# GatorSense/HyperPRI

Hardware: AMD Instinct MI355X
Metric: HSI cubes/sec (608x968x238) fwd+bwd (higher is better)
Workload: dtype f32; 1 GPU; CubeNET-64 n_channels=238 HSI 608x968 fp32, per-GPU batch 2, train mode, BCEWithLogits, fwd+bwd; global_batch=2, parallelism=dp1

## Files before the change

### hyperpri_amd/csrc/conv_wino.hip

```cpp
#include "common.h"

extern "C" size_t hpri_wino_packed_floats(int K, int Ncols_pad) { return (size_t)hpri_cdiv(K, 8) * 16 * 8 * Ncols_pad; }

struct WinoWgradArgs {
  const float* x; int x_cs, x_coff, x_cvalid;
  const float* dy; int dy_cs, dy_coff, dy_cvalid;
  float* ws;
  int N, H, W, Cr, Nr, cblk;
  int strips_x, strips_y, total, per_split;
  int ntile, items, per_xcd;
  int kw;
};

#define WG_XROW 36
#define WG_X_BYTES (4 * WG_XROW * 256)
#define WG_Y_BYTES (2 * 32 * 256)
#define WG_STAGE_BYTES (WG_X_BYTES + WG_Y_BYTES)

__global__ __launch_bounds__(512, 2) void conv_wino_wgrad_kernel(WinoWgradArgs a) {
  __shared__ __attribute__((aligned(1024))) unsigned char smem[2 * WG_STAGE_BYTES];
  const int tid = threadIdx.x, lane = tid & 63, wave = __builtin_amdgcn_readfirstlane(tid >> 6);
  const int li = lane & 31, lh = lane >> 5;
  const int fa = wave >> 1, fb = wave & 1;
  const int item = (int)(blockIdx.x & 7) * a.per_xcd + (int)(blockIdx.x >> 3);
  if (item >= a.items) return;
  const int split = item / a.ntile, tile = item - split * a.ntile;
  const int cb = tile % a.cblk, nbk = tile / a.cblk;
  const int c_blk = cb * 64, n_blk = nbk * 64;
  const int u0 = split * a.per_split, u1 = min(a.total, u0 + a.per_split);

  const int r1 = (fa == 0) ? 0 : 1, r2 = (fa == 3) ? 3 : 2;
  const float s1 = (fa == 2) ? -1.f : 1.f, s2 = (fa == 1 || fa == 2) ? 1.f : -1.f;
  const int c0 = fb;
  const float sigma = s1 * s2;

  f32x16 acc[2][2][2];
#pragma unroll
  for (int e = 0; e < 2; ++e)
#pragma unroll
    for (int ct = 0; ct < 2; ++ct)
#pragma unroll
      for (int nt = 0; nt < 2; ++nt)
#pragma unroll
        for (int r = 0; r < 16; ++r) acc[e][ct][nt][r] = 0.f;

  constexpr int NPX = 4 * (WG_XROW / 4), NPY = 2 * 8, NPW = (NPX + NPY + 7) / 8;
  constexpr unsigned OOB = 0xFFFFFFF0u;
  const int l4 = lane >> 4;
  const unsigned xlane = (c_blk + (lane & 15) * 4 < a.x_cvalid) ? (unsigned)(l4 * a.x_cs * 4 + (lane & 15) * 16) : OOB;
  const unsigned ylane = (n_blk + (lane & 15) * 4 < a.dy_cvalid) ? (unsigned)(l4 * a.dy_cs * 4 + (lane & 15) * 16) : OOB;
#define LOAD_UNIT(u_, buf_)                                                                                            \
  {                                                                                                                    \
    int q_ = (u_);                                                                                                     \
    const int sx_ = q_ % a.strips_x; q_ /= a.strips_x;                                                                 \
    const int sy_ = q_ % a.strips_y; const int img_ = q_ / a.strips_y;                                                 \
    const int y0_ = sy_ * 2, x0_ = sx_ * 32;                                                                           \
    kend_next = min(8, (a.kw - x0_ + 3) >> 2);                                \
    unsigned char* lb_ = smem + (buf_) * WG_STAGE_BYTES;                                                               \
    const float* xu_ = a.x + ((long long)(img_ * a.H + y0_ - 1) * a.W + x0_ - 1) * a.x_cs + a.x_coff + c_blk;          \
    const float* yu_ = a.dy + ((long long)(img_ * a.H + y0_) * a.W + x0_) * a.dy_cs + a.dy_coff + n_blk;               \
    const hpri_rsrc_t rx_ = HPRI_MAKE_RSRC(xu_, 0x7FFFFF00);       \
    const hpri_rsrc_t ry_ = HPRI_MAKE_RSRC(yu_, 0x7FFFFF00);       \
    _Pragma("unroll") for (int p = 0; p < NPW; ++p) {                                                                  \
      const int piece_ = p * 8 + wave;                                                                                 \
      if (piece_ < NPX) {                                                                                              \
        const int row_ = piece_ / (WG_XROW / 4), pxb_ = (piece_ % (WG_XROW / 4)) * 4;                 \
        const bool rowok_ = (unsigned)(y0_ + row_ - 1) < (unsigned)a.H;                                                \
        const bool ok_ = rowok_ && (pxb_ + l4) < 34 && (unsigned)(x0_ + pxb_ + l4 - 1) < (unsigned)a.W;                \
        HPRI_LDS_DMA16(rx_, lb_ + piece_ * 1024, ok_ ? xlane : OOB, (row_ * a.W + pxb_) * a.x_cs * 4);           \
      } else if (piece_ < NPX + NPY) {                                                                                 \
        const int pp_ = piece_ - NPX;                                                                                  \
        const int row_ = pp_ >> 3, pxb_ = (pp_ & 7) * 4;                                                               \
        const bool ok_ = (y0_ + row_) < a.H && (x0_ + pxb_ + l4) < a.W;                                                \
        HPRI_LDS_DMA16(ry_, lb_ + piece_ * 1024, ok_ ? ylane : OOB, (row_ * a.W + pxb_) * a.dy_cs * 4);          \
      }                                                                                                                \
    }                                                                                                                  \
  }

#define K_STEP(FA_, FB_)                                               \
    {                                                                                                                  \
      const int tile = 2 * kk + lh;                                                                                    \
      float va[2][2], vb[2][2];                                               \
      _Pragma("unroll") for (int ct = 0; ct < 2; ++ct) {                                                               \
        float P[3];                                                                                                    \
        _Pragma("unroll") for (int c = 0; c < 3; ++c) {                                                                \
          const float d1 = xs[(r1 * WG_XROW + 2 * tile + c0 + c) * 64 + ct * 32 + li];                                 \
          const float d2 = xs[(r2 * WG_XROW + 2 * tile + c0 + c) * 64 + ct * 32 + li];                                 \
          P[c] = d1 + sigma * d2;                                                                                      \
        }                                                                                                              \
        va[0][ct] = FB_ ? (P[1] - P[0]) : (P[0] - P[2]);                                                               \
        va[1][ct] = FB_ ? (P[0] - P[2]) : (P[1] + P[2]);                                                               \
      }                                                                                                                \
      _Pragma("unroll") for (int nt = 0; nt < 2; ++nt) {                                                               \
        float t0, t1;                                                                                                  \
        if (FA_ == 0 || FA_ == 3) {                                                                                    \
          t0 = ys[(((FA_ == 3) ? 1 : 0) * 32 + 2 * tile + 0) * 64 + nt * 32 + li];                                     \
          t1 = ys[(((FA_ == 3) ? 1 : 0) * 32 + 2 * tile + 1) * 64 + nt * 32 + li];                                     \
        } else {                                                                                                       \
          const float y00 = ys[(0 * 32 + 2 * tile + 0) * 64 + nt * 32 + li], y01 = ys[(0 * 32 + 2 * tile + 1) * 64 + nt * 32 + li]; \
          const float y10 = ys[(1 * 32 + 2 * tile + 0) * 64 + nt * 32 + li], y11 = ys[(1 * 32 + 2 * tile + 1) * 64 + nt * 32 + li]; \
          t0 = (FA_ == 1) ? (y00 + y10) : (y00 - y10);                                                                 \
          t1 = (FA_ == 1) ? (y01 + y11) : (y01 - y11);                                                                 \
        }                                                                                                              \
        vb[0][nt] = FB_ ? (t0 - t1) : t0;                                                                              \
        vb[1][nt] = FB_ ? t1 : (t0 + t1);                                                                              \
      }                                                                                                                \
      _Pragma("unroll") for (int e = 0; e < 2; ++e)                                                                    \
          _Pragma("unroll") for (int ct = 0; ct < 2; ++ct)                                                             \
              _Pragma("unroll") for (int nt = 0; nt < 2; ++nt)                                                         \
                  acc[e][ct][nt] = __builtin_amdgcn_mfma_f32_32x32x2f32(va[e][ct], vb[e][nt], acc[e][ct][nt], 0, 0, 0); \
    }
#define UNIT_LOOP(FA_, FB_)                                                                                            \
  for (int u = u0; u < u1; ++u) {                                                                                      \
    asm volatile("s_waitcnt vmcnt(0)" ::: "memory");                                                                   \
    __builtin_amdgcn_s_barrier();                     \
    const int kend = kend_next;                                                                                        \
    if (u + 1 < u1) LOAD_UNIT(u + 1, (u + 1 - u0) & 1)                                                                 \
    const float* xs = reinterpret_cast<const float*>(smem + ((u - u0) & 1) * WG_STAGE_BYTES);                          \
    const float* ys = xs + WG_X_BYTES / 4;                                                                             \
    _Pragma("unroll 2") for (int kk = 0; kk < kend; ++kk) K_STEP(FA_, FB_)                                             \
  }
  int kend_next = 8;
  if (u0 < u1) LOAD_UNIT(u0, 0)
  switch (wave) {
    case 0: UNIT_LOOP(0, 0) break;
    case 1: UNIT_LOOP(0, 1) break;
    case 2: UNIT_LOOP(1, 0) break;
    case 3: UNIT_LOOP(1, 1) break;
    case 4: UNIT_LOOP(2, 0) break;
    case 5: UNIT_LOOP(2, 1) break;
    case 6: UNIT_LOOP(3, 0) break;
    default: UNIT_LOOP(3, 1) break;
  }
#undef UNIT_LOOP
#undef K_STEP
#undef LOAD_UNIT
  float* slab = a.ws + (size_t)split * 16 * a.Cr * a.Nr;
  const float sdy = (fa == 3) ? -s1 : s1;
  const float sgn[2] = {sdy, (fb == 1) ? -sdy : sdy};
#pragma unroll
  for (int e = 0; e < 2; ++e) {
    const int xi = fa * 4 + 2 * fb + e;
#pragma unroll
    for (int ct = 0; ct < 2; ++ct)
#pragma unroll
      for (int nt = 0; nt < 2; ++nt) {
        const int n = n_blk + nt * 32 + li;
#pragma unroll
        for (int r = 0; r < 16; ++r) {
          const int c = c_blk + ct * 32 + (r & 3) + 8 * (r >> 2) + 4 * lh;
          slab[((size_t)xi * a.Cr + c) * a.Nr + n] = sgn[e] * acc[e][ct][nt][r];
        }
      }
  }
}

__global__ void wino_wgrad_reduce_kernel(const float* __restrict__ ws, float* __restrict__ dw, int splits, int Cr, int Nr,
                                         int Cin, int Cout, int accumulate) {
  const int n = blockIdx.x * 64 + (threadIdx.x & 63), c = blockIdx.y * 4 + (threadIdx.x >> 6);
  if (n >= Cout || c >= Cin) return;
  float u[16];
#pragma unroll
  for (int xi = 0; xi < 16; ++xi) u[xi] = 0.f;
  const size_t slab = (size_t)16 * Cr * Nr;
  for (int k = 0; k < splits; ++k) {
    const float* p = ws + (size_t)k * slab + (size_t)c * Nr + n;
#pragma unroll
    for (int xi = 0; xi < 16; ++xi) u[xi] += p[(size_t)xi * Cr * Nr];
  }
  float t[3][4];
#pragma unroll
  for (int j = 0; j < 4; ++j) {
    t[0][j] = u[0 * 4 + j] + 0.5f * (u[1 * 4 + j] + u[2 * 4 + j]);
    t[1][j] = 0.5f * (u[1 * 4 + j] - u[2 * 4 + j]);
    t[2][j] = 0.5f * (u[1 * 4 + j] + u[2 * 4 + j]) + u[3 * 4 + j];
  }
  float* o = dw + ((size_t)n * Cin + c) * 9;
#pragma unroll
  for (int i = 0; i < 3; ++i) {
    const float g0 = t[i][0] + 0.5f * (t[i][1] + t[i][2]), g1 = 0.5f * (t[i][1] - t[i][2]), g2 = 0.5f * (t[i][1] + t[i][2]) + t[i][3];
    o[i * 3 + 0] = accumulate ? o[i * 3 + 0] + g0 : g0;
    o[i * 3 + 1] = accumulate ? o[i * 3 + 1] + g1 : g1;
    o[i * 3 + 2] = accumulate ? o[i * 3 + 2] + g2 : g2;
  }
}

constexpr int wino_wide_cols(int S) { return S >= 16 ? 32 : 64; }

template <int S>
__global__ __launch_bounds__(wino_wide_cols(S) * S) void wino_wgrad_reduce_wide_kernel(const float* __restrict__ ws,
                                                                                       float* __restrict__ dw, int splits, int Cr,
                                                                                       int Nr, int Cin, int Cout, int accumulate) {
  constexpr int NC = wino_wide_cols(S);
  __shared__ float red[S - 1][16][NC];
  const int ln = threadIdx.x % NC, sl = threadIdx.x / NC;
  const int n = blockIdx.x * NC + ln, c = blockIdx.y;
  float u[16];
#pragma unroll
  for (int xi = 0; xi < 16; ++xi) u[xi] = 0.f;
  const size_t slab = (size_t)16 * Cr * Nr;
#pragma unroll 1
  for (int k = sl; k < splits; k += S) {
    const float* p = ws + (size_t)k * slab + (size_t)c * Nr + n;
#pragma unroll
    for (int xi = 0; xi < 16; ++xi) u[xi] += p[(size_t)xi * Cr * Nr];
  }
  if (sl > 0) {
#pragma unroll
    for (int xi = 0; xi < 16; ++xi) red[sl - 1][xi][ln] = u[xi];
  }
  __syncthreads();
  if (sl > 0 || n >= Cout) return;
#pragma unroll 2
  for (int q = 0; q < S - 1; ++q)
#pragma unroll
    for (int xi = 0; xi < 16; ++xi) u[xi] += red[q][xi][ln];
  float t[3][4];
#pragma unroll
  for (int j = 0; j < 4; ++j) {
    t[0][j] = u[0 * 4 + j] + 0.5f * (u[1 * 4 + j] + u[2 * 4 + j]);
    t[1][j] = 0.5f * (u[1 * 4 + j] - u[2 * 4 + j]);
    t[2][j] = 0.5f * (u[1 * 4 + j] + u[2 * 4 + j]) + u[3 * 4 + j];
  }
  float* o = dw + ((size_t)n * Cin + c) * 9;
#pragma unroll
  for (int i = 0; i < 3; ++i) {
    const float g0 = t[i][0] + 0.5f * (t[i][1] + t[i][2]), g1 = 0.5f * (t[i][1] - t[i][2]), g2 = 0.5f * (t[i][1] + t[i][2]) + t[i][3];
    o[i * 3 + 0] = accumulate ? o[i * 3 + 0] + g0 : g0;
    o[i * 3 + 1] = accumulate ? o[i * 3 + 1] + g1 : g1;
    o[i * 3 + 2] = accumulate ? o[i * 3 + 2] + g2 : g2;
  }
}

extern "C" int hpri_wino_wgrad_plan(int N, int H, int W, int Cin_pad, int Cout_pad, int* splits, int* Cr, int* Nr) {
  const int cblk = hpri_cdiv(Cin_pad, 64), nblk = hpri_cdiv(Cout_pad, 64);
  const int total = N * hpri_cdiv(H, 2) * hpri_cdiv(W, 32);
  *Cr = cblk * 64; *Nr = nblk * 64;
  const int tiles = cblk * nblk;
  auto plan = [&](int cus, int kmax, double tol) {
    int best = 1; double best_eff = 0.0;
    for (int k = 1; k <= kmax; ++k) {
      if (k > 1 && total / k < 8) break;
      const double per_cu = (double)tiles * k / (double)cus;
      double eff = per_cu / (double)((long long)(per_cu + 0.999999));
      if (per_cu < 1.0) eff = per_cu;
      if (eff > best_eff + tol + 1e-9) { best_eff = eff; best = k; }
    }
    return best;
  };
  int best = plan(256, 512, 0.0);
  const int reserve = hpri_option(5);
  if (reserve > 0) best = plan(256 - (reserve < 192 ? reserve : 192), 2 * best, 0.05);
  *splits = best;
  return HPRI_OK;
}

extern "C" int hpri_conv_wino_wgrad(const float* x, int x_cs, int x_coff, int x_cvalid, const float* dy, int dy_cs, int dy_coff,
                                    int dy_cvalid, float* ws, size_t ws_floats, int N, int H, int W, int Cin_pad, int Cout_pad,
                                    hipStream_t stream) {
  HPRI_REQUIRE(x && dy && ws, "conv_wino_wgrad: null pointer");
  HPRI_REQUIRE(N > 0 && H > 0 && W > 0 && Cin_pad > 0 && Cout_pad > 0, "conv_wino_wgrad: bad sizes");
  HPRI_REQUIRE(x_cs % 4 == 0 && x_coff % 4 == 0 && dy_cs % 4 == 0 && dy_coff % 4 == 0 && x_cvalid % 4 == 0 && dy_cvalid % 4 == 0,
               "conv_wino_wgrad: channel strides / offsets / valid counts must be multiples of 4");
  HPRI_REQUIRE(((uintptr_t)x & 15) == 0 && ((uintptr_t)dy & 15) == 0, "conv_wino_wgrad: pointers must be 16-byte aligned");
  HPRI_REQUIRE((long long)5 * W * x_cs * 4 < (1ll << 31) && (long long)3 * W * dy_cs * 4 < (1ll << 31),
               "conv_wino_wgrad: image rows too long for 32-bit buffer offsets");
  WinoWgradArgs a;
  a.x = x; a.x_cs = x_cs; a.x_coff = x_coff; a.x_cvalid = x_cvalid; a.dy = dy; a.dy_cs = dy_cs; a.dy_coff = dy_coff; a.dy_cvalid = dy_cvalid;
  a.ws = ws; a.N = N; a.H = H; a.W = W;
  int splits;
  hpri_wino_wgrad_plan(N, H, W, Cin_pad, Cout_pad, &splits, &a.Cr, &a.Nr);
  if ((size_t)splits * 16 * a.Cr * a.Nr > ws_floats) return hpri_set_error(HPRI_ERR_WORKSPACE, "conv_wino_wgrad: workspace too small");
  a.cblk = a.Cr / 64;
  a.strips_x = hpri_cdiv(W, 32); a.strips_y = hpri_cdiv(H, 2); a.total = N * a.strips_x * a.strips_y;
  a.per_split = hpri_cdiv(a.total, splits);
  a.ntile = a.cblk * (a.Nr / 64);
  a.items = splits * a.ntile; a.per_xcd = hpri_cdiv(a.items, 8);
  a.kw = hpri_option(6) != 0 ? W : a.strips_x * 32;
  dim3 grid((unsigned)(a.per_xcd * 8), 1u, 1u);
  hipLaunchKernelGGL(conv_wino_wgrad_kernel, grid, dim3(512), 0, stream, a);
  HPRI_CHECK_LAUNCH();
  return HPRI_OK;
}

extern "C" int hpri_wino_wgrad_reduce(const float* ws, float* dw, int N, int H, int W, int Cin, int Cin_pad, int Cout, int Cout_pad,
                                      int accumulate, hipStream_t stream) {
  HPRI_REQUIRE(ws && dw && Cin > 0 && Cout > 0, "wino_wgrad_reduce: bad arguments");
  int splits, Cr, Nr;
  hpri_wino_wgrad_plan(N, H, W, Cin_pad, Cout_pad, &splits, &Cr, &Nr);
  if (splits >= 64) {
    dim3 grid((unsigned)hpri_cdiv(Cout, wino_wide_cols(16)), (unsigned)Cin);
    hipLaunchKernelGGL(wino_wgrad_reduce_wide_kernel<16>, grid, dim3(wino_wide_cols(16) * 16), 0, stream, ws, dw, splits, Cr, Nr, Cin, Cout, accumulate);
  } else if (splits >= 8) {
    dim3 grid((unsigned)hpri_cdiv(Cout, 64), (unsigned)Cin);
    hipLaunchKernelGGL(wino_wgrad_reduce_wide_kernel<8>, grid, dim3(512), 0, stream, ws, dw, splits, Cr, Nr, Cin, Cout, accumulate);
  } else {
    dim3 grid((unsigned)hpri_cdiv(Cout, 64), (unsigned)hpri_cdiv(Cin, 4));
    hipLaunchKernelGGL(wino_wgrad_reduce_kernel, grid, dim3(256), 0, stream, ws, dw, splits, Cr, Nr, Cin, Cout, accumulate);
  }
  HPRI_CHECK_LAUNCH();
  return HPRI_OK;
}
```

Baseline: 65.72 cubes/s.

## Vectorize Winograd wgrad LDS reads with interleaved channel pairs and pinned scheduling

Reworks the Winograd weight-gradient inner step so each lane reads adjacent channel pairs from LDS as 8-byte vectors through a running byte pointer. The transform signs and row choices become compile-time constants per wave. Channels are remapped to interleaved pairs so the output slab can be written with paired stores, and strip indices are advanced incrementally instead of recomputed with divisions. Inline-asm pins and a sched_barrier fix the placement of the transform arithmetic before the MFMAs. The aim is fewer LDS instructions and less address arithmetic, at the risk of worse compiler scheduling or register pressure.

```diff
diff --git a/hyperpri_amd/csrc/conv_wino.hip b/hyperpri_amd/csrc/conv_wino.hip
--- a/hyperpri_amd/csrc/conv_wino.hip
+++ b/hyperpri_amd/csrc/conv_wino.hip
@@ -1,4 +1,6 @@
 #include "common.h"
+
+typedef float f32x2 __attribute__((ext_vector_type(2)));
 
 extern "C" size_t hpri_wino_packed_floats(int K, int Ncols_pad) { return (size_t)hpri_cdiv(K, 8) * 16 * 8 * Ncols_pad; }
 
@@ -29,10 +31,7 @@
   const int c_blk = cb * 64, n_blk = nbk * 64;
   const int u0 = split * a.per_split, u1 = min(a.total, u0 + a.per_split);
 
-  const int r1 = (fa == 0) ? 0 : 1, r2 = (fa == 3) ? 3 : 2;
-  const float s1 = (fa == 2) ? -1.f : 1.f, s2 = (fa == 1 || fa == 2) ? 1.f : -1.f;
-  const int c0 = fb;
-  const float sigma = s1 * s2;
+  const float s1 = (fa == 2) ? -1.f : 1.f;
 
   f32x16 acc[2][2][2];
 #pragma unroll
@@ -49,11 +48,11 @@
   const int l4 = lane >> 4;
   const unsigned xlane = (c_blk + (lane & 15) * 4 < a.x_cvalid) ? (unsigned)(l4 * a.x_cs * 4 + (lane & 15) * 16) : OOB;
   const unsigned ylane = (n_blk + (lane & 15) * 4 < a.dy_cvalid) ? (unsigned)(l4 * a.dy_cs * 4 + (lane & 15) * 16) : OOB;
-#define LOAD_UNIT(u_, buf_)                                                                                            \
+  int ld_sx = u0 % a.strips_x, ld_sy = (u0 / a.strips_x) % a.strips_y, ld_img = u0 / (a.strips_x * a.strips_y);
+#define LOAD_UNIT(buf_)                                                                                                \
   {                                                                                                                    \
-    int q_ = (u_);                                                                                                     \
-    const int sx_ = q_ % a.strips_x; q_ /= a.strips_x;                                                                 \
-    const int sy_ = q_ % a.strips_y; const int img_ = q_ / a.strips_y;                                                 \
+    const int sx_ = ld_sx, sy_ = ld_sy, img_ = ld_img;                                                                 \
+    if (++ld_sx == a.strips_x) { ld_sx = 0; if (++ld_sy == a.strips_y) { ld_sy = 0; ++ld_img; } }                      \
     const int y0_ = sy_ * 2, x0_ = sx_ * 32;                                                                           \
     kend_next = min(8, (a.kw - x0_ + 3) >> 2);                                \
     unsigned char* lb_ = smem + (buf_) * WG_STAGE_BYTES;                                                               \
@@ -79,49 +78,72 @@
 
 #define K_STEP(FA_, FB_)                                               \
     {                                                                                                                  \
-      const int tile = 2 * kk + lh;                                                                                    \
+      constexpr int R1_ = (FA_ == 0) ? 0 : 1, R2_ = (FA_ == 3) ? 3 : 2;              \
+      constexpr int YR_ = (FA_ == 3) ? 1 : 0, YROWS_ = (FA_ == 1 || FA_ == 2) ? 2 : 1;                                 \
+      asm("" : "+v"(kp));                               \
+      f32x2 d[2][3], y[2][2];                                          \
+      _Pragma("unroll") for (int c = 0; c < 3; ++c) {                                                                  \
+        d[0][c] = WG_LDS2(kp + (R1_ * WG_XROW + FB_ + c) * 256);                                                       \
+        d[1][c] = WG_LDS2(kp + (R2_ * WG_XROW + FB_ + c) * 256);                                                       \
+      }                                                                                                                \
+      _Pragma("unroll") for (int r = 0; r < YROWS_; ++r)                                                               \
+        _Pragma("unroll") for (int px = 0; px < 2; ++px) y[r][px] = WG_LDS2(kp + WG_X_BYTES + ((YR_ + r) * 32 + px) * 256); \
       float va[2][2], vb[2][2];                                               \
+      float P[3][2];                                                                                                   \
+      _Pragma("unroll") for (int c = 0; c < 3; ++c)                                                                    \
+        _Pragma("unroll") for (int ct = 0; ct < 2; ++ct) {                                                             \
+          float d1_ = d[0][c][ct], d2_ = d[1][c][ct];                                                                  \
+          WG_PIN(d1_) WG_PIN(d2_)                                                                                      \
+          P[c][ct] = (FA_ == 1) ? (d1_ + d2_) : (d1_ - d2_);                                        \
+          WG_PIN(P[c][ct])                                                                                             \
+        }                                                                                                              \
       _Pragma("unroll") for (int ct = 0; ct < 2; ++ct) {                                                               \
-        float P[3];                                                                                                    \
-        _Pragma("unroll") for (int c = 0; c < 3; ++c) {                                                                \
-          const float d1 = xs[(r1 * WG_XROW + 2 * tile + c0 + c) * 64 + ct * 32 + li];                                 \
-          const float d2 = xs[(r2 * WG_XROW + 2 * tile + c0 + c) * 64 + ct * 32 + li];                                 \
-          P[c] = d1 + sigma * d2;                                                                                      \
+        va[0][ct] = FB_ ? (P[1][ct] - P[0][ct]) : (P[0][ct] - P[2][ct]);                                               \
+        va[1][ct] = FB_ ? (P[0][ct] - P[2][ct]) : (P[1][ct] + P[2][ct]);                                               \
+                                                                                                                       \
+      }                                                                                                                \
+      float t[2][2];                                                               \
+      _Pragma("unroll") for (int px = 0; px < 2; ++px)                                                                 \
+        _Pragma("unroll") for (int nt = 0; nt < 2; ++nt) {                                                             \
+          float y0_ = y[0][px][nt];                                                                                    \
+          WG_PIN(y0_)                                                                                                  \
+          if (YROWS_ == 2) {                                                                                           \
+            float y1_ = y[1][px][nt];                                                                                  \
+            WG_PIN(y1_)                                                                                                \
+            y0_ = (FA_ == 1) ? (y0_ + y1_) : (y0_ - y1_);                                                              \
+            WG_PIN(y0_)                                                                                                \
+          }                                                                                                            \
+          t[px][nt] = y0_;                                                                                             \
         }                                                                                                              \
-        va[0][ct] = FB_ ? (P[1] - P[0]) : (P[0] - P[2]);                                                               \
-        va[1][ct] = FB_ ? (P[0] - P[2]) : (P[1] + P[2]);                                                               \
+      _Pragma("unroll") for (int nt = 0; nt < 2; ++nt) {                                                               \
+        vb[0][nt] = FB_ ? (t[0][nt] - t[1][nt]) : t[0][nt];                                                            \
+        vb[1][nt] = FB_ ? t[1][nt] : (t[0][nt] + t[1][nt]);                                                            \
+                                                                                                                       \
       }                                                                                                                \
-      _Pragma("unroll") for (int nt = 0; nt < 2; ++nt) {                                                               \
-        float t0, t1;                                                                                                  \
-        if (FA_ == 0 || FA_ == 3) {                                                                                    \
-          t0 = ys[(((FA_ == 3) ? 1 : 0) * 32 + 2 * tile + 0) * 64 + nt * 32 + li];                                     \
-          t1 = ys[(((FA_ == 3) ? 1 : 0) * 32 + 2 * tile + 1) * 64 + nt * 32 + li];                                     \
-        } else {                                                                                                       \
-          const float y00 = ys[(0 * 32 + 2 * tile + 0) * 64 + nt * 32 + li], y01 = ys[(0 * 32 + 2 * tile + 1) * 64 + nt * 32 + li]; \
-          const float y10 = ys[(1 * 32 + 2 * tile + 0) * 64 + nt * 32 + li], y11 = ys[(1 * 32 + 2 * tile + 1) * 64 + nt * 32 + li]; \
-          t0 = (FA_ == 1) ? (y00 + y10) : (y00 - y10);                                                                 \
-          t1 = (FA_ == 1) ? (y01 + y11) : (y01 - y11);                                                                 \
-        }                                                                                                              \
-        vb[0][nt] = FB_ ? (t0 - t1) : t0;                                                                              \
-        vb[1][nt] = FB_ ? t1 : (t0 + t1);                                                                              \
-      }                                                                                                                \
+      __builtin_amdgcn_sched_barrier(0);                            \
       _Pragma("unroll") for (int e = 0; e < 2; ++e)                                                                    \
           _Pragma("unroll") for (int ct = 0; ct < 2; ++ct)                                                             \
               _Pragma("unroll") for (int nt = 0; nt < 2; ++nt)                                                         \
                   acc[e][ct][nt] = __builtin_amdgcn_mfma_f32_32x32x2f32(va[e][ct], vb[e][nt], acc[e][ct][nt], 0, 0, 0); \
+      kp += 1024;                                                                           \
     }
 #define UNIT_LOOP(FA_, FB_)                                                                                            \
   for (int u = u0; u < u1; ++u) {                                                                                      \
     asm volatile("s_waitcnt vmcnt(0)" ::: "memory");                                                                   \
     __builtin_amdgcn_s_barrier();                     \
     const int kend = kend_next;                                                                                        \
-    if (u + 1 < u1) LOAD_UNIT(u + 1, (u + 1 - u0) & 1)                                                                 \
-    const float* xs = reinterpret_cast<const float*>(smem + ((u - u0) & 1) * WG_STAGE_BYTES);                          \
-    const float* ys = xs + WG_X_BYTES / 4;                                                                             \
-    _Pragma("unroll 2") for (int kk = 0; kk < kend; ++kk) K_STEP(FA_, FB_)                                             \
-  }
+    if (u + 1 < u1) LOAD_UNIT((u + 1 - u0) & 1)                                                                         \
+    unsigned kp = ((u - u0) & 1) * WG_STAGE_BYTES + klane;                                                             \
+    for (int kk = 0; kk < kend; ++kk) K_STEP(FA_, FB_)                                                                 \
+  }
+  const unsigned klane = (unsigned)(lh * 512 + li * 8);
+  typedef __attribute__((address_space(3))) const unsigned char* wg_lds_bytes;
+  typedef __attribute__((address_space(3))) const volatile f32x2* wg_lds_f32x2;
+  const wg_lds_bytes lds = (wg_lds_bytes)smem;
+#define WG_LDS2(off_) (*(wg_lds_f32x2)(lds + (off_)))
+#define WG_PIN(v_) asm("" : "+v"(v_));
   int kend_next = 8;
-  if (u0 < u1) LOAD_UNIT(u0, 0)
+  if (u0 < u1) LOAD_UNIT(0)
   switch (wave) {
     case 0: UNIT_LOOP(0, 0) break;
     case 1: UNIT_LOOP(0, 1) break;
@@ -135,6 +157,8 @@
 #undef UNIT_LOOP
 #undef K_STEP
 #undef LOAD_UNIT
+#undef WG_LDS2
+#undef WG_PIN
   float* slab = a.ws + (size_t)split * 16 * a.Cr * a.Nr;
   const float sdy = (fa == 3) ? -s1 : s1;
   const float sgn[2] = {sdy, (fb == 1) ? -sdy : sdy};
@@ -144,13 +168,12 @@
 #pragma unroll
     for (int ct = 0; ct < 2; ++ct)
 #pragma unroll
-      for (int nt = 0; nt < 2; ++nt) {
-        const int n = n_blk + nt * 32 + li;
-#pragma unroll
-        for (int r = 0; r < 16; ++r) {
-          const int c = c_blk + ct * 32 + (r & 3) + 8 * (r >> 2) + 4 * lh;
-          slab[((size_t)xi * a.Cr + c) * a.Nr + n] = sgn[e] * acc[e][ct][nt][r];
-        }
+      for (int r = 0; r < 16; ++r) {
+        const int c = c_blk + 2 * ((r & 3) + 8 * (r >> 2) + 4 * lh) + ct;
+        f32x2 o;
+        o[0] = sgn[e] * acc[e][ct][0][r];
+        o[1] = sgn[e] * acc[e][ct][1][r];
+        *reinterpret_cast<f32x2*>(&slab[((size_t)xi * a.Cr + c) * a.Nr + n_blk + 2 * li]) = o;
       }
   }
 }
```

Result: faster. 67.07 cubes/s, median of 6 (+2.1%).
